# TRI-ML/packnet-sfm

Measured on AMD Instinct MI355X. Metric: images/sec PackNet01 self-sup train 192x640, higher is better.
Workload: dtype f32; 1 GPU; PackNet01(1A)+PoseNet self-supervised train step (fwd+photometric loss+bwd+allreduce+Adam), KITTI-shaped 192x640 triplets, batch 4/GPU (BASELINE.json configs[1]); global_batch=4, parallelism=dp1, wgrad_side_stream=True, pose_branch_stream=True, tuning=shipped database (346 decisions) + autotune for unlisted shapes, step_launch=eager, devices_visible=1

## Files before the change

include/pnsfm.h:

```cpp
#ifndef PNSFM_H
#define PNSFM_H

#include <stddef.h>
#include <stdint.h>

#ifdef __cplusplus
extern "C" {
#endif

int pnsfm_version(void);
const char* pnsfm_last_error(void);
const char* pnsfm_build_target(void);

size_t pnsfm_conv2d_packed_elems_fwd(int Cin, int Cout, int ks);
size_t pnsfm_conv2d_packed_elems_bwd(int Cin, int Cout, int ks);
int pnsfm_conv2d_pack_weights(const float* w, float* wp_fwd , float* wp_bwd ,
                              int Cin, int Cout, int ks, void* stream);
size_t pnsfm_conv2d_pack_item_bytes(void);
int pnsfm_conv2d_pack_item_fill(void* item_host, const float* w, float* wp_fwd, float* wp_bwd, int Cin, int Cout, int ks,
                                int first_block);
int pnsfm_conv2d_pack_table(const void* table_dev, int n_items, int total_blocks, void* stream);
int pnsfm_conv2d_forward(const float* x, const float* wp_fwd, const float* bias , float* y,
                         int B, int Cin, int Cout, int H, int W, int ks, void* stream);
int pnsfm_conv2d_backward_data(const float* dy, const float* wp_bwd, float* dx,
// ... 128 lines not shown
#define PNSFM_MAX_REGION_OPS 12
typedef struct {
  const float* src;
  float* dst;
  int n[4];
  long long src_stride[4];
  long long dst_stride[4];
  int op;
} pnsfm_region_op;
int pnsfm_region_ops(const void* ops_host, int n_ops, void* stream);

int pnsfm_upsample_nearest_forward(const float* x, float* y, int N, int h, int w, int s, void* stream);
int pnsfm_upsample_nearest_backward(const float* dy, float* dx, int N, int h, int w, int s, void* stream);

int pnsfm_loss_combine_forward(const float* const* photometric, int n, const float* const* smoothness, int ns, float weight,
                               float* out3, void* stream);
int pnsfm_loss_combine_backward(const float* g, int n, int ns, float weight, float* dout16, void* stream);

int pnsfm_pack_bias_eff_forward(const float* W2, const float* b2, const float* b3, float* Ssum, float* bias_eff, int C, int d,
                                int blk, void* stream);
int pnsfm_pack_bias_eff_backward(const float* g, const float* Ssum, const float* b3, const float* dWeff_full, float* db3, float* dW2,
                                 int C, int d, int D, int k, void* stream);

int pnsfm_adam_step(float* param, const float* grad, float* exp_avg, float* exp_avg_sq, size_t n,
                    float lr, float beta1, float beta2, float eps, float weight_decay, float grad_scale,
                    int step, void* stream);
int pnsfm_adam_flat_step(float* param, const float* grad, float* exp_avg, float* exp_avg_sq, size_t n, float* hp, void* stream);
int pnsfm_adam_flat_update(float* param, const float* grad, float* exp_avg, float* exp_avg_sq, size_t n, float* hp, int tick,
                           void* stream);
size_t pnsfm_adam_pack_item_bytes(void);
int pnsfm_adam_pack_item_fill(void* item_host, float* w, const float* g, float* m, float* v, const float* hp, float* wp_fwd,
                              float* wp_bwd, int Cin, int Cout, int ks, int first_block);
int pnsfm_adam_pack_table(const void* table_dev, int n_items, int total_blocks, void* stream);
size_t pnsfm_adam_seg_bytes(void);
int pnsfm_adam_seg_fill(void* seg_host, float* p, const float* g, float* m, float* v, const float* hp, size_t n, int first_block);
int pnsfm_adam_segments(const void* segs_dev, int nseg, int total_blocks, void* stream);

int pnsfm_stream_wait_stream(void* waiter, void* signaler);
int pnsfm_calib_mfma(float* sink, int blocks, int iters, void* stream);
int pnsfm_calib_copy(const float* src, float* dst, size_t n_floats, void* stream);
int pnsfm_prof_enable(int on);
int pnsfm_prof_reset(void);
int pnsfm_prof_collect(int kind, double* total_ms, double* total_flops, long long* launches);
int pnsfm_prof_dump(const char* path);

size_t pnsfm_sparse_compact_ws_ints(int ncell);
// ... 69 lines not shown
```

packnet-sfm_amd/csrc/api.hip:

```cpp
#include "pnsfm_common.h"
#include "../../include/pnsfm.h"

#include <cstdarg>
#include <cstdio>
#include <mutex>
#include <cstdlib>
#include <utility>
#include <vector>

namespace pnsfm {

static thread_local char g_err[512] = "";

void set_error(const char* fmt, ...) {
  va_list ap;
  va_start(ap, fmt);
  vsnprintf(g_err, sizeof(g_err), fmt, ap);
  va_end(ap);
}

int check_launch(const char* what) {
  int e = (int)hipGetLastError();
  if (e != 0) {
    set_error("%s: launch failed: %s", what, hipGetErrorString((hipError_t)e));
// ... 173 lines not shown
  if (hipGetDevice(&cur) != hipSuccess) { pnsfm::set_error("stream_wait_stream: hipGetDevice failed"); return -1; }
  const int dev = device_of(signaler, cur), dw = device_of(waiter, dev);
  if (dev < 0 || dev >= 64) { pnsfm::set_error("stream_wait_stream: bad device %d", dev); return -1; }
  if (dw != dev) { pnsfm::set_error("stream_wait_stream: the two streams live on different devices (%d, %d)", dw, dev); return -1; }
  struct DevGuard { int prev, now; DevGuard(int p, int n) : prev(p), now(n) { if (p != n) (void)hipSetDevice(n); } ~DevGuard() { if (prev != now) (void)hipSetDevice(prev); } } guard(cur, dev);
  hipEvent_t ev;
  {
    std::lock_guard<std::mutex> lk(mu);
    auto& r = ring[dev];
    if (r.size() < 256) {
      if (hipEventCreateWithFlags(&ev, hipEventDisableTiming) != hipSuccess) { pnsfm::set_error("stream_wait_stream: hipEventCreate failed"); return -1; }
      r.push_back(ev);
    } else {
      ev = r[next[dev]];
      next[dev] = (next[dev] + 1) % 256;
    }
  }
  if (hipEventRecord(ev, (hipStream_t)signaler) != hipSuccess) { pnsfm::set_error("stream_wait_stream: hipEventRecord failed"); return -1; }
  if (hipStreamWaitEvent((hipStream_t)waiter, ev, 0) != hipSuccess) { pnsfm::set_error("stream_wait_stream: hipStreamWaitEvent failed"); return -1; }
  return 0;
#endif
}

int pnsfm_prof_enable(int on) {
#ifndef PNSFM_EMU
  std::lock_guard<std::mutex> lk(pnsfm::g_prof_mu);
  pnsfm::g_prof_on = on != 0;
#else
  (void)on;
#endif
  return 0;
}

int pnsfm_prof_reset(void) {
#ifndef PNSFM_EMU
  std::lock_guard<std::mutex> lk(pnsfm::g_prof_mu);
  for (int k = 0; k < 2; ++k) {
    for (auto& r : pnsfm::g_recs[k]) {
      hipEventSynchronize(r.b);
      pnsfm::g_pool.push_back(r.a);
      pnsfm::g_pool.push_back(r.b);
    }
    pnsfm::g_recs[k].clear();
  }
#endif
  return 0;
// ... 43 lines not shown
```

packnet-sfm_amd/csrc/seq/pnsfm_seq.cpp:

```cpp
#include <torch/extension.h>

#include <cstdint>
#include <string>
#include <vector>

#include "../../../include/pnsfm.h"

namespace {

struct Abi {
  decltype(&pnsfm_last_error) last_error = nullptr;
  decltype(&pnsfm_conv2d_forward) conv2d_forward = nullptr;
  decltype(&pnsfm_conv2d_forward_cat) conv2d_forward_cat = nullptr;
  decltype(&pnsfm_conv2d_backward_data) conv2d_backward_data = nullptr;
  decltype(&pnsfm_conv2d_backward_data_add) conv2d_backward_data_add = nullptr;
  decltype(&pnsfm_conv2d_backward_weight) conv2d_backward_weight = nullptr;
  decltype(&pnsfm_conv2d_backward_weight_cat) conv2d_backward_weight_cat = nullptr;
  decltype(&pnsfm_groupnorm_act_forward) groupnorm_act_forward = nullptr;
  decltype(&pnsfm_groupnorm_act_backward) groupnorm_act_backward = nullptr;
  decltype(&pnsfm_stream_wait_stream) stream_wait_stream = nullptr;
  decltype(&pnsfm_region_ops) region_ops = nullptr;
  bool require_cuda = true;
  bool bound = false;
} g;

template <class F>
void take(F& slot, const py::dict& d, const char* name) {
  if (!d.contains(name)) throw std::runtime_error(std::string("pnsfm_seq.bind: missing symbol ") + name);
  slot = reinterpret_cast<F>(static_cast<uintptr_t>(d[name].cast<uint64_t>()));
}

void bind(const py::dict& addrs, bool require_cuda) {
  take(g.last_error, addrs, "pnsfm_last_error");
  take(g.conv2d_forward, addrs, "pnsfm_conv2d_forward");
  take(g.conv2d_forward_cat, addrs, "pnsfm_conv2d_forward_cat");
  take(g.conv2d_backward_data, addrs, "pnsfm_conv2d_backward_data");
  take(g.conv2d_backward_data_add, addrs, "pnsfm_conv2d_backward_data_add");
  take(g.conv2d_backward_weight, addrs, "pnsfm_conv2d_backward_weight");
  take(g.conv2d_backward_weight_cat, addrs, "pnsfm_conv2d_backward_weight_cat");
  take(g.groupnorm_act_forward, addrs, "pnsfm_groupnorm_act_forward");
  take(g.groupnorm_act_backward, addrs, "pnsfm_groupnorm_act_backward");
  take(g.stream_wait_stream, addrs, "pnsfm_stream_wait_stream");
  take(g.region_ops, addrs, "pnsfm_region_ops");
  g.require_cuda = require_cuda;
  g.bound = true;
}

void rc_check(int rc, const char* what) {
  if (rc != 0) throw std::runtime_error(std::string(what) + " failed (rc=" + std::to_string(rc) + "): " + (g.last_error ? g.last_error() : "?"));
}

void chk(const at::Tensor& t, const char* what, const at::Tensor* ref = nullptr) {
  if (g.require_cuda && !t.is_cuda())
    throw std::runtime_error(std::string("packnet_sfm HIP op got a ") + t.device().str() + " tensor (" + what +
                             "): the HIP kernels run on MI355X only, there is no CPU fallback");
  if (t.scalar_type() != at::kFloat) throw std::runtime_error(std::string("packnet_sfm HIP op needs float32 tensors (") + what + ")");
  if (!t.is_contiguous()) throw std::runtime_error(std::string("packnet_sfm HIP op needs contiguous tensors (") + what + ")");
  if (ref && t.device() != ref->device()) throw std::runtime_error("packnet_sfm HIP op got tensors on different devices");
}
const float* cptr(const at::Tensor& t) { return t.data_ptr<float>(); }
const float* cptr(const c10::optional<at::Tensor>& t) { return (t.has_value() && t->defined()) ? t->data_ptr<float>() : nullptr; }
float* mptr(at::Tensor& t) { return t.data_ptr<float>(); }
void* sp(uint64_t s) { return reinterpret_cast<void*>(static_cast<uintptr_t>(s)); }

void launch_conv_fwd(const std::vector<at::Tensor>& xs, const at::Tensor& wp, const c10::optional<at::Tensor>& bias, at::Tensor& y,
                     int Cout, int ks, uint64_t stream) {
// ... 203 lines not shown
      const auto& src = std::get<2>(it);
      const bool has_src = src.has_value() && src->defined();
      if (dst.scalar_type() != at::kFloat || (has_src && src->scalar_type() != at::kFloat)) throw std::runtime_error("region_ops needs float32 tensors");
      if (g.require_cuda && !dst.is_cuda())
        throw std::runtime_error("packnet_sfm HIP op got a " + dst.device().str() + " tensor: the HIP kernels run on MI355X only, there is no CPU fallback");
      if (dst.dim() > 4 || (has_src && src->sizes() != dst.sizes()) || dst.device() != ref.device())
        throw std::runtime_error("region_ops: windows must be <= 4-D, of equal shape, on one device");
      const int pad = 4 - (int)dst.dim();
      arr[k].dst = dst.data_ptr<float>();
      arr[k].src = has_src ? src->data_ptr<float>() : nullptr;
      arr[k].op = (int)std::get<0>(it);
      for (int d = 0; d < 4; ++d) {
        const int64_t nd = d < pad ? 1 : dst.size(d - pad);
        if (nd == 0) throw std::runtime_error("region_ops: empty window");
        arr[k].n[d] = (int)nd;
        arr[k].dst_stride[d] = d < pad ? 0 : dst.stride(d - pad);
        arr[k].src_stride[d] = (!has_src || d < pad) ? 0 : src->stride(d - pad);
      }
    }
    rc_check(g.region_ops(arr, (int)n, sp(stream)), "region_ops");
  }
}

}

PYBIND11_MODULE(TORCH_EXTENSION_NAME, m) {
  m.doc() = "packnet_sfm block sequencer: bodies of the hot autograd nodes as single calls over the C ABI of libpnsfm_hip.so";
  m.def("bind", &bind, py::arg("addresses"), py::arg("require_cuda"));
  m.def("conv_gn_act_forward", &conv_gn_act_forward);
  m.def("conv_gn_act_backward", &conv_gn_act_backward);
  m.def("conv2d_forward", &conv2d_forward);
  m.def("conv2d_backward", &conv2d_backward);
  m.def("gn_act_forward", &gn_act_forward);
  m.def("gn_act_backward", &gn_act_backward);
  m.def("region_ops", &region_ops);
}
```

packnet-sfm_amd/packnet_sfm/hip/_lib.py:

```python
import ctypes
import os

import torch

_HERE = os.path.dirname(os.path.abspath(__file__))
_CSRC = os.path.abspath(os.path.join(_HERE, "..", "..", "csrc"))
LIB_PATH = os.path.join(_CSRC, "libpnsfm_hip.so")

_p = ctypes.c_void_p
_i = ctypes.c_int
_f = ctypes.c_float
_sz = ctypes.c_size_t
_ll = ctypes.c_longlong
_d = ctypes.c_double

SIGNATURES = {
    "pnsfm_version": (_i, []),
    "pnsfm_last_error": (ctypes.c_char_p, []),
    "pnsfm_build_target": (ctypes.c_char_p, []),
    "pnsfm_conv2d_packed_elems_fwd": (_sz, [_i, _i, _i]),
    "pnsfm_conv2d_packed_elems_bwd": (_sz, [_i, _i, _i]),
    "pnsfm_conv2d_pack_weights": (_i, [_p, _p, _p, _i, _i, _i, _p]),
    "pnsfm_conv2d_pack_item_bytes": (_sz, []),
    "pnsfm_conv2d_pack_item_fill": (_i, [_p, _p, _p, _p, _i, _i, _i, _i]),
# ... 15 lines not shown
    "pnsfm_groupnorm_act_backward": (_i, [_p, _p, _p, _p, _p, _p, _p, _p, _p, _p, _p, _i, _i, _i, _i, _i, _p]),
    "pnsfm_set_gn_fused": (_i, [_i]),
    "pnsfm_space_to_depth": (_i, [_p, _p, _i, _i, _i, _i, _sz, _p]),
    "pnsfm_depth_to_space": (_i, [_p, _p, _i, _i, _i, _i, _p]),
    "pnsfm_conv3d_forward": (_i, [_p, _p, _p, _p, _i, _i, _i, _i, _i, _p]),
    "pnsfm_conv3d_backward_data": (_i, [_p, _p, _p, _i, _i, _i, _i, _i, _p]),
    "pnsfm_conv3d_backward_weight": (_i, [_p, _p, _p, _p, _p, _i, _i, _i, _i, _i, _p]),
    "pnsfm_set_pack3d_fold": (_i, [_i]),
    "pnsfm_conv3d_d2s_folded": (_i, [_p, _p, _i, _i]),
    "pnsfm_conv3d_forward_d2s": (_i, [_p, _p, _p, _p, _p, _i, _i, _i, _i, _i, _p]),
    "pnsfm_conv3d_rows_folded": (_i, [_p, _p, _i]),
    "pnsfm_conv3d_forward_rows": (_i, [_p, _p, _p, _p, _i, _i, _i, _i, _i, _i, _p]),
    "pnsfm_conv3d_backward_data_rows": (_i, [_p, _p, _p, _i, _i, _i, _i, _i, _i, _p]),
    "pnsfm_conv3d_backward_weight_rows": (_i, [_p, _p, _p, _p, _i, _i, _i, _i, _i, _i, _p]),
    "pnsfm_invdepth_act_forward": (_i, [_p, _p, _sz, _f, _p]),
    "pnsfm_invdepth_act_backward": (_i, [_p, _p, _p, _sz, _f, _p]),
    "pnsfm_pose_vec2mat_forward": (_i, [_p, _p, _i, _p]),
    "pnsfm_upsample_nearest_forward": (_i, [_p, _p, _i, _i, _i, _i, _p]),
    "pnsfm_upsample_nearest_backward": (_i, [_p, _p, _i, _i, _i, _i, _p]),
    "pnsfm_loss_combine_forward": (_i, [_p, _i, _p, _i, _f, _p, _p]),
    "pnsfm_loss_combine_backward": (_i, [_p, _i, _i, _f, _p, _p]),
    "pnsfm_pack_bias_eff_forward": (_i, [_p, _p, _p, _p, _p, _i, _i, _i, _p]),
    "pnsfm_pack_bias_eff_backward": (_i, [_p, _p, _p, _p, _p, _p, _i, _i, _i, _i, _p]),
    "pnsfm_pose_vec2mat_backward": (_i, [_p, _p, _p, _i, _p]),
    "pnsfm_supervised_loss_forward": (_i, [_p, _p, _p, _p, _sz, _i, _i, _p]),
    "pnsfm_supervised_loss_backward": (_i, [_p, _p, _p, _p, _p, _sz, _i, _i, _p]),
    "pnsfm_invdepth_conv_forward": (_i, [_p, _p, _p, _p, _i, _i, _i, _i, _f, _p]),
    "pnsfm_invdepth_conv_backward": (_i, [_p, _p, _p, _p, _p, _p, _i, _i, _i, _i, _p]),
    "pnsfm_view_synthesis_forward": (_i, [_p, _p, _p, _p, _p, _p, _i, _i, _i, _i, _i, _p]),
    "pnsfm_view_synthesis_backward": (_i, [_p, _p, _p, _p, _p, _p, _p, _p, _i, _i, _i, _i, _i, _p]),
    "pnsfm_photometric_forward": (_i, [_p, _p, _p, _p, _p, _p, _i, _i, _i, _i, _f, _f, _f, _i, _i, _f, _p]),
    "pnsfm_photometric_backward": (_i, [_p, _p, _p, _p, _f, _p, _i, _i, _i, _i, _f, _f, _f, _i, _i, _i, _p]),
    "pnsfm_smoothness_norm_forward": (_i, [_p, _p, _p, _p, _i, _i, _i, _p]),
    "pnsfm_smoothness_norm_backward": (_i, [_p, _p, _p, _p, _p, _i, _i, _i, _p]),
    "pnsfm_region_ops": (_i, [_p, _i, _p]),
    "pnsfm_conv2d_packed_elems_h16": (_sz, [_i, _i, _i]),
    "pnsfm_set_h16_max_split": (_i, [_i]),
    "pnsfm_conv2d_pack_weights_h16": (_i, [_p, _i, _p, _i, _i, _i, _p]),
    "pnsfm_conv2d_forward_h16": (_i, [_p, _i, _p, _i, _p, _i, _p, _p, _p, _i, _i, _i, _i, _i, _p]),
    "pnsfm_groupnorm_act_forward_h16": (_i, [_p, _p, _p, _p, _p, _p, _p, _i, _i, _i, _i, _f, _i, _p]),
    "pnsfm_conv3d_forward_h16": (_i, [_p, _p, _p, _p, _i, _i, _i, _i, _i, _p]),
    "pnsfm_space_to_depth_h16": (_i, [_p, _p, _i, _i, _i, _i, _p]),
    "pnsfm_depth_to_space_h16": (_i, [_p, _p, _i, _i, _i, _i, _p]),
    "pnsfm_upsample_nearest_forward_h16": (_i, [_p, _p, _i, _i, _i, _i, _p]),
    "pnsfm_invdepth_conv_forward_h16": (_i, [_p, _p, _p, _p, _i, _i, _i, _i, _f, _p]),
    "pnsfm_region_ops_h16": (_i, [_p, _i, _p]),
# ... 104 lines not shown
```

packnet-sfm_amd/packnet_sfm/hip/_seq.py:

```python
import ctypes
import importlib.util
import os

from . import _lib

_HERE = os.path.dirname(os.path.abspath(__file__))
SEQ_PATH = os.path.join(_HERE, "_pnsfm_seq.so")
_SYMBOLS = ("pnsfm_last_error", "pnsfm_conv2d_forward", "pnsfm_conv2d_forward_cat", "pnsfm_conv2d_backward_data",
            "pnsfm_conv2d_backward_data_add", "pnsfm_conv2d_backward_weight", "pnsfm_conv2d_backward_weight_cat",
            "pnsfm_groupnorm_act_forward", "pnsfm_groupnorm_act_backward", "pnsfm_stream_wait_stream", "pnsfm_region_ops")
_ON = os.environ.get("PNSFM_SEQ", "1") != "0"
_MOD = None
_BOUND = None


def set_enabled(on):
    global _ON
    _ON = bool(on)


def enabled():
    return _ON


def _load():
    global _MOD
    if _MOD is None:
        if not os.path.exists(SEQ_PATH):
            raise ImportError("%s not found -- build it with `python __graft_entry__.py` (packnet-sfm_amd/csrc/build.py: build_seq); "
                              "PNSFM_SEQ=0 runs the pure-Python bodies instead" % SEQ_PATH)
        spec = importlib.util.spec_from_file_location("_pnsfm_seq", SEQ_PATH)
        mod = importlib.util.module_from_spec(spec)
        spec.loader.exec_module(mod)
# ... 16 lines not shown
```

packnet-sfm_amd/packnet_sfm/hip/functional.py:

```python
import contextlib
import os
import weakref

import torch
from torch.autograd import Function
from torch.autograd.function import once_differentiable

from . import ops
from . import _seq
from ._lib import HipError as _HipError

_WEIGHT_EPOCH = [0]


def bump_weight_epoch():
    _WEIGHT_EPOCH[0] += 1


def get_conv_math():
    from . import _lib
    return 'bx3' if _lib.get().pnsfm_get_conv_math() else 'f32'


def set_conv_math(mode):
# ... 862 lines not shown
        return Weff

    @staticmethod
    @once_differentiable
    def backward(ctx, g):
        W2pad, w3 = ctx.saved_tensors
        g = g.contiguous()
        _WgradStream.side_ok(*ctx.params)
        dW2 = dW3 = None
        if ctx.needs_input_grad[0]:
            dW2 = ops.conv3d_forward(g, w3, torch.zeros(w3.shape[0], device=g.device, dtype=g.dtype))[:, :, 1:-1, 1:-1].contiguous()
        if ctx.needs_input_grad[1]:
            dW3, _ = ops.conv3d_backward_weight(g, W2pad)
        return dW2, dW3, None


def compose_pack_weight(W2, W3):
    return ComposePackWeightFn.apply(W2, W3, torch.is_grad_enabled())


class ComposePackParamsFn(Function):

    @staticmethod
    def forward(ctx, W2, b2, W3, b3, recording=True):
        W2d, w3, b3d = W2.detach().contiguous(), W3.detach().contiguous(), b3.detach().contiguous()
        W2pad = torch.nn.functional.pad(W2d, (1, 1, 1, 1))
        Weff = ops.conv3d_backward_data(W2pad, w3)
        bias_eff, Ssum = ops.pack_bias_eff_forward(W2d, None if b2 is None else b2.detach().contiguous(), b3d)
        ctx.save_for_backward(W2pad, w3, b3d, Ssum)
        ctx.params = (W2, W3)
        ctx.k = W2.shape[-1]
        _WgradStream.note_use(recording, W2, W3)
        return Weff, bias_eff

    @staticmethod
    @once_differentiable
    def backward(ctx, gW, gb):
        W2pad, w3, b3, Ssum = ctx.saved_tensors
        _WgradStream.side_ok(*ctx.params)
        need_W2, need_b2, need_W3, need_b3 = ctx.needs_input_grad[:4]
        C = W2pad.shape[0]
        if gW is None:
            gW = W2pad.new_zeros((C, W2pad.shape[1] // w3.shape[0], ctx.k + 2, ctx.k + 2))
        if gb is None:
            gb = W2pad.new_zeros((C,))
        gW, gb = gW.contiguous(), gb.contiguous()
        dW2 = dW3 = db3 = None
        if need_W2 or need_b3:
            full = ops.conv3d_forward(gW, w3, None) if need_W2 else W2pad
            db3, dW2 = ops.pack_bias_eff_backward(gb, Ssum, b3, full, ctx.k, want_db3=need_b3, want_dW2=need_W2)
        if need_W3:
            dW3, _ = ops.conv3d_backward_weight(gW, W2pad)
        return dW2, (gb if need_b2 else None), dW3, db3, None


def compose_pack_params(W2, b2, W3, b3):
    return ComposePackParamsFn.apply(W2, b2, W3, b3, torch.is_grad_enabled())


def _R(op, dst, src=None):
    return (op, dst, src)


def _border_split_fwd(P, S, lr_t, run):
    B, C, h, w = P.shape
    tb = P.new_empty((2 * B, C, S, w))
    lr = P.new_empty((2 * B, C, S, h)) if lr_t else P.new_empty((2 * B, C, h, S))
    lrv = lr.transpose(2, 3) if lr_t else lr
    run([_R(ops.REGION_COPY, tb[:B], P[:, :, :S]), _R(ops.REGION_COPY, tb[B:], P[:, :, h - S:]),
         _R(ops.REGION_COPY, lrv[:B], P[:, :, :, :S]), _R(ops.REGION_COPY, lrv[B:], P[:, :, :, w - S:])])
    return tb, lr


def _strip_select_fwd(z, B, r, dim, run):
    n2 = 2 * r
    if dim == 2:
        out = z.new_empty((z.shape[0], z.shape[1], n2, z.shape[3]))
        run([_R(ops.REGION_COPY, out[:B], z[:B, :, :n2]), _R(ops.REGION_COPY, out[B:], z[B:, :, 1:])])
    else:
        out = z.new_empty((z.shape[0], z.shape[1], z.shape[2], n2))
# ... 792 lines not shown
```

packnet-sfm_amd/packnet_sfm/hip/ops.py:

```python
import ctypes
import threading

import torch

from . import _lib


try:
    _raw_stream = torch._C._cuda_getCurrentRawStream
except AttributeError:
    _raw_stream = None


_TLS = threading.local()


class stream_override:

    def __init__(self, raw, device_index=None):
        self.ov = (raw, device_index)

    def __enter__(self):
        self.prev = getattr(_TLS, 'ov', None)
        _TLS.ov = self.ov
# ... 1223 lines not shown
        chunk = items[i0:i0 + MAX_REGION_OPS]
        arr = (_RegionOp * len(chunk))()
        for k, (op, dst, src) in enumerate(chunk):
            if dst.dtype != torch.float32 or (src is not None and src.dtype != torch.float32):
                raise RuntimeError("region_ops needs float32 tensors")
            if _lib.REQUIRE_CUDA and not dst.is_cuda:
                raise RuntimeError("packnet_sfm HIP op got a %s tensor: the HIP kernels run on MI355X only, there is no CPU fallback" % dst.device)
            if dst.dim() > 4 or (src is not None and tuple(src.shape) != tuple(dst.shape)) or dst.device != ref.device:
                raise RuntimeError("region_ops: windows must be <= 4-D, of equal shape, on one device")
            pad = 4 - dst.dim()
            shape = (1,) * pad + tuple(dst.shape)
            if 0 in shape:
                raise RuntimeError("region_ops: empty window")
            arr[k].dst = dst.data_ptr()
            arr[k].src = src.data_ptr() if src is not None else None
            arr[k].op = int(op)
            for d in range(4):
                arr[k].n[d] = shape[d]
                arr[k].dst_stride[d] = 0 if d < pad else dst.stride(d - pad)
                arr[k].src_stride[d] = 0 if (src is None or d < pad) else src.stride(d - pad)
        _lib.check(_lib.get().pnsfm_region_ops(ctypes.byref(arr), len(chunk), _stream(ref)), "region_ops")



def _h16(*tensors):
    for t in tensors:
        if t is not None and t.dtype != torch.float16:
            raise RuntimeError("packnet_sfm fp16 HIP op needs float16 tensors, got %s" % t.dtype)


def conv2d_pack_h16(w, out=None):
    _chk(w, out)
    if w.dtype not in (torch.float16, torch.float32):
        raise RuntimeError("conv2d_pack_h16: weight must be float16 or float32, got %s" % w.dtype)
    Cout, Cin, ks, _ = w.shape
    n = int(_lib.get().pnsfm_conv2d_packed_elems_h16(Cin, Cout, ks))
    if out is None or out.numel() != n or out.device != w.device:
        out = torch.empty(n, dtype=torch.float16, device=w.device)
    _h16(out)
    _lib.check(_lib.get().pnsfm_conv2d_pack_weights_h16(_ptr(w), 1 if w.dtype == torch.float32 else 0, _ptr(out), Cin, Cout, ks,
                                                         _stream(w)), "conv2d_pack_weights_h16")
    return out


def conv2d_forward_h16(xs, wp, bias, Cout, ks):
    xs = tuple(xs)
# ... 138 lines not shown
```

packnet-sfm_amd/packnet_sfm/networks/depth/PackNet01.py:

```python
import torch
import torch.nn as nn

from packnet_sfm.hip import functional as HF
from packnet_sfm.networks.layers.packnet.layers01 import Conv2D, InvDepth, PackLayerConv3d, ResidualBlock, UnpackLayerConv3d


class PackNet01(nn.Module):

    STEM_WIDTH = 64
    WIDTHS = (64, 64, 128, 256, 512)
    NUM_3D_FEAT = 8

    def __init__(self, dropout=None, version=None, **kwargs):
        super().__init__()
        if version is None or version[1:] not in ('A', 'B'):
            raise ValueError('Unknown PackNet version {}'.format(version))
        self.version = version[1:]
        concat = self.version == 'A'
        ni, no = self.STEM_WIDTH, 1
        n = list(self.WIDTHS)
        d3 = self.NUM_3D_FEAT
        blocks = [2, 2, 3, 3]
        pack_k = [5, 3, 3, 3, 3]
        if concat:
            dec_out = list(n)
            dec_in = [n[0] + ni + no, n[1] + n[0] + no, n[2] + n[1] + no, n[3] + n[2], n[4] + n[3]]
        else:
# ... 9 lines not shown
        unpack_in = [n[1], n[2], n[3], n[4], n[4]]
        for i in (4, 3, 2, 1, 0):
            setattr(self, 'unpack%d' % (i + 1), UnpackLayerConv3d(unpack_in[i], dec_out[i], 3, d=d3))
        for i in (4, 3, 2, 1, 0):
            setattr(self, 'iconv%d' % (i + 1), Conv2D(dec_in[i], n[i], 3, 1))
        for i in (3, 2, 1, 0):
            setattr(self, 'disp%d_layer' % (i + 1), InvDepth(n[i], out_channels=no))
        self.init_weights()

    def init_weights(self):
        for m in self.modules():
            if isinstance(m, (nn.Conv2d, nn.Conv3d)):
                nn.init.xavier_uniform_(m.weight)
                if m.bias is not None:
                    m.bias.data.zero_()

    def _merge(self, up, skip, disp=None):
        parts = (up, skip) if self.version == 'A' else (up + skip,)
        if disp is not None:
            parts = parts + (HF.upsample_nearest(disp, scale_factor=2),)
        return parts if len(parts) > 1 else parts[0]

    def forward(self, rgb):
        x = self.pre_calc(rgb)
        c1, x_s = self.conv1.forward_tap(x)
        x1p = self.pack1(c1)
        c2, x1p_s = self.conv2.forward_tap(x1p)
        x2p = self.pack2(c2)
        c3, x2p_s = self.conv3.forward_tap(x2p)
        x3p = self.pack3(c3)
        c4, x3p_s = self.conv4.forward_tap(x3p)
        x4p = self.pack4(c4)
        c5, x4p_s = self.conv5.forward_tap(x4p)
        x5p = self.pack5(c5)

        iconv5 = self.iconv5(self._merge(self.unpack5(x5p), x4p_s))
        iconv4 = self.iconv4(self._merge(self.unpack4(iconv5), x3p_s))
        up3, iconv4_t = self.unpack3.forward_tap(iconv4)
        disp4 = self.disp4_layer(iconv4_t)
        iconv3 = self.iconv3(self._merge(up3, x2p_s, disp4))
        up2, iconv3_t = self.unpack2.forward_tap(iconv3)
        disp3 = self.disp3_layer(iconv3_t)
        iconv2 = self.iconv2(self._merge(up2, x1p_s, disp3))
        up1, iconv2_t = self.unpack1.forward_tap(iconv2)
        disp2 = self.disp2_layer(iconv2_t)
        iconv1 = self.iconv1(self._merge(up1, x_s, disp2))
# ... 10 lines not shown
```

packnet-sfm_amd/packnet_sfm/networks/depth/PackNetSAN01.py:

```python
import torch
import torch.nn as nn

from packnet_sfm.hip import functional as HF
from packnet_sfm.networks.layers.minkowski_encoder import MinkowskiEncoder
from packnet_sfm.networks.layers.packnet.layers01 import Conv2D, InvDepth, PackLayerConv3d, ResidualBlock, UnpackLayerConv3d


class Encoder(nn.Module):
    def __init__(self, version, in_channels, ni, n1, n2, n3, n4, n5, pack_kernel, num_blocks, num_3d_feat, dropout):
        super().__init__()
        self.version = version
        n = [n1, n2, n3, n4, n5]
        self.pre_calc = Conv2D(in_channels, ni, 5, 1)
        for i in range(5):
            setattr(self, 'pack%d' % (i + 1), PackLayerConv3d(n[i], pack_kernel[i], d=num_3d_feat))
        self.conv1 = Conv2D(ni, n1, 7, 1)
        for i in range(4):
            setattr(self, 'conv%d' % (i + 2), ResidualBlock(n[i], n[i + 1], num_blocks[i], 1, dropout=dropout))

    def forward(self, rgb):
        x = self.pre_calc(rgb)
        x1p = self.pack1(self.conv1(x))
        x2p = self.pack2(self.conv2(x1p))
        x3p = self.pack3(self.conv3(x2p))
        x4p = self.pack4(self.conv4(x3p))
        x5p = self.pack5(self.conv5(x4p))
        return x5p, [x, x1p, x2p, x3p, x4p]


class Decoder(nn.Module):
    def __init__(self, version, out_channels, ni, n1, n2, n3, n4, n5, unpack_kernel, iconv_kernel, num_3d_feat):
        super().__init__()
        self.version = version
        n = [n1, n2, n3, n4, n5]
        nin = [n1 + ni + out_channels, n2 + n1 + out_channels, n3 + n2 + out_channels, n4 + n3, n5 + n4]
        unpack_in = [n2, n3, n4, n5, n5]
        for j, i in enumerate((4, 3, 2, 1, 0)):
            setattr(self, 'unpack%d' % (i + 1), UnpackLayerConv3d(unpack_in[i], n[i], unpack_kernel[j], d=num_3d_feat))
        for j, i in enumerate((4, 3, 2, 1, 0)):
            setattr(self, 'iconv%d' % (i + 1), Conv2D(nin[i], n[i], iconv_kernel[j], 1))
        self.unpack_disps = nn.PixelShuffle(2)
        self.unpack_disp4 = nn.Upsample(scale_factor=2, mode='nearest')
        self.unpack_disp3 = nn.Upsample(scale_factor=2, mode='nearest')
# ... 73 lines not shown
```

packnet-sfm_amd/packnet_sfm/networks/layers/packnet/layers01.py:

```python
import torch
import torch.nn as nn
import torch.nn.functional as F

from packnet_sfm.hip import functional as HF
from packnet_sfm.hip import ops as _ops


class _HipConv2d(nn.Conv2d):

    def __init__(self, in_channels, out_channels, kernel_size, stride=1):
        if stride != 1:
            raise NotImplementedError('the gfx950 conv kernel implements stride 1 only (all PackNet01 convs)')
        super().__init__(in_channels, out_channels, kernel_size=kernel_size, stride=stride)
        self._packed = HF.PackedConvWeight()

    def forward(self, x):
        if isinstance(x, (tuple, list)):
            return HF.conv2d_cat(tuple(x), self.weight, self.bias, self._packed)
        return HF.conv2d(x, self.weight, self.bias, self._packed)

    def forward_tap(self, x):
        return HF.conv2d_tap(x, self.weight, self.bias, self._packed)


# ... 103 lines not shown
        if r != 2:
            raise NotImplementedError('r=2 only')
        self.conv = Conv2D(in_channels, out_channels * (r ** 2), kernel_size, 1)

    def forward(self, x):
        return HF.depth_to_space(self.conv(x))


class PackLayerConv3d(nn.Module):

    collapse = 'auto'
    lr_transposed = True
    strip_frame_rows = True

    def __init__(self, in_channels, kernel_size, r=2, d=8):
        super().__init__()
        if r != 2 or d not in (4, 8):
            raise NotImplementedError('the gfx950 packing kernels implement r=2 and d in {4, 8} (PackNet01 / PackNetSlim01)')
        self.d = d
        self.conv = Conv2D(in_channels * (r ** 2) * d, in_channels, kernel_size, 1)
        self.conv3d = nn.Conv3d(1, d, kernel_size=(3, 3, 3), stride=(1, 1, 1), padding=(1, 1, 1))
        self._eff_packed = HF.PackedConvWeight(volatile=True)
        self._lr_packed = HF.PackedConvWeight()

    def _use_collapsed(self, h, w):
        k = self.conv.kernel_size
        r = k // 2
        if h < 2 * r + 1 or w < 2 * r + 1 or self.collapse is False:
            return False
        if self.collapse is True:
            return True
        orig = float(self.d) * k * k * h * w
        strips = float(self.d) * k * k * (2 * (2 * r) * w + 2 * h * (2 * r))
        return (k + 2) ** 2 * h * w + strips <= 0.7 * orig

    def _conv_reference_form(self, P):
        feats = HF.conv3d_1to8(P, self.conv3d.weight, self.conv3d.bias)
        return self.conv.conv_base(feats)

    def _conv_collapsed_h16(self, P):
        base = self.conv.conv_base
        W2, b2, W3, b3 = base.weight, base.bias, self.conv3d.weight, self.conv3d.bias
        HF._h16_params(W2, b2, W3, b3)
        return HF._h16_run(lambda P, *params: self._collapsed_h16_body(P), P, W2, b2, W3, b3)

    def _collapsed_h16_body(self, P):
        base = self.conv.conv_base
        W2, b2, W3, b3 = base.weight, base.bias, self.conv3d.weight, self.conv3d.bias
        key = tuple(None if t is None else HF.PackedConvWeight.key_of(t) for t in (W2, b2, W3, b3))
        with torch.no_grad():
            if self._eff_packed.key_h16 != key:
                W_eff, bias_eff = HF.compose_pack_params(W2.float(), None if b2 is None else b2.float(), W3.float(), b3.float())
                self._eff_packed.get_h16(W_eff, bias_eff, key=key, hold=(W2, b2, W3, b3))
            k = self.conv.kernel_size
            r, S = k // 2, 2 * (k // 2) + 1
            B = P.shape[0]
            lr_t = bool(self.lr_transposed)
            P_main, tb, lr = HF.pack_border_split(P, S, lr_t)
            y = HF.conv2d_h16_composed(P_main, None, None, self._eff_packed, key)
            o_tb = base(HF.strip_select(HF.conv3d_1to8(tb, W3, b3), B, r, 2))
            if lr_t:
                z = HF.conv3d_1to8(lr, W3.transpose(3, 4), b3)
                o_lr = HF.conv2d(HF.strip_select(z, B, r, 2), W2.transpose(2, 3), b2, self._lr_packed)
            else:
                o_lr = base(HF.strip_select(HF.conv3d_1to8(lr, W3, b3), B, r, 3))
            return HF.pack_border_paste(y, o_tb, o_lr, r, lr_t)

    def _conv_collapsed(self, P):
        if P.dtype == torch.float16:
            return self._conv_collapsed_h16(P)
        base = self.conv.conv_base
        W2, b2, W3, b3 = base.weight, base.bias, self.conv3d.weight, self.conv3d.bias
        k = self.conv.kernel_size
        r, S = k // 2, 2 * (k // 2) + 1
        B, _, h, w = P.shape
        W_eff, bias_eff = HF.compose_pack_params(W2, b2, W3, b3)
        lr_t = bool(self.lr_transposed)
        rows = bool(self.strip_frame_rows)
        P_main, tb, lr = HF.pack_border_split(P, S, lr_t)
        y = HF.conv2d(P_main, W_eff, bias_eff, self._eff_packed)
        s_tb = HF.conv3d_1to8_rows(tb, W3, b3, B, r)
        o_tb = HF.conv2d_rows(s_tb, W2, b2, base._packed, r) if rows else base(s_tb)
        if lr_t:
            z = HF.conv3d_1to8_rows(lr, W3.transpose(3, 4), b3, B, r)
            o_lr = (HF.conv2d_rows(z, W2.transpose(2, 3), b2, self._lr_packed, r) if rows else
                    HF.conv2d(z, W2.transpose(2, 3), b2, self._lr_packed))
        else:
            o_lr = base(HF.strip_select(HF.conv3d_1to8(lr, W3, b3), B, r, 3))
        return HF.pack_border_paste(y, o_tb, o_lr, r, lr_t, rows)

    def forward(self, x):
        P = HF.space_to_depth(x)
        y = self._conv_collapsed(P) if self._use_collapsed(P.shape[2], P.shape[3]) else self._conv_reference_form(P)
        norm = self.conv.normalize
        return HF.groupnorm_act(y, norm.weight, norm.bias, 16, norm.eps, _ops.ACT_ELU)


class UnpackLayerConv3d(nn.Module):

    def __init__(self, in_channels, out_channels, kernel_size, r=2, d=8):
        super().__init__()
        if r != 2 or d not in (4, 8):
            raise NotImplementedError('the gfx950 unpacking kernels implement r=2 and d in {4, 8} (PackNet01 / PackNetSlim01)')
        self.conv = Conv2D(in_channels, out_channels * (r ** 2) // d, kernel_size, 1)
        self.conv3d = nn.Conv3d(1, d, kernel_size=(3, 3, 3), stride=(1, 1, 1), padding=(1, 1, 1))

    def forward(self, x):
        return HF.conv3d_1to8_d2s(self.conv(x), self.conv3d.weight, self.conv3d.bias)

    def forward_tap(self, x):
        y, x_tap = self.conv.forward_tap(x)
        return HF.conv3d_1to8_d2s(y, self.conv3d.weight, self.conv3d.bias), x_tap


from packnet_sfm._merge import reference_fallback as _reference_fallback
__getattr__ = _reference_fallback(__name__, __file__)
```

Baseline: 178.6 images/sec.

## Precompute collapsed pack-layer weights on side stream at forward start

Adds a fused host entry point that pads W2, composes the effective weight and bias, and packs the forward/backward conv weights for each PackLayerConv3d in one call. At the start of the network forward these are issued for all pack layers on the wgrad side stream, and each layer waits on an event only just before its main conv. This moves per-layer weight composition and packing off the critical launch path so it overlaps with earlier layers. It adds persistent buffers and cross-stream dependencies, and relies on the layer's previous-call collapsed flag, so the first step takes the old path.

```diff
diff --git a/include/pnsfm.h b/include/pnsfm.h
--- a/include/pnsfm.h
+++ b/include/pnsfm.h
@@ -174,6 +174,24 @@
 int pnsfm_pack_bias_eff_backward(const float* g, const float* Ssum, const float* b3, const float* dWeff_full, float* db3, float* dW2,
                                  int C, int d, int D, int k, void* stream);
 
+typedef struct {
+  const float* W2;
+  const float* b2;
+  const float* W3;
+  const float* b3;
+  int C, D, d, k;
+  float* W2pad;
+  float* Weff;
+  float* bias_eff;
+  float* Ssum;
+  float* eff_fwd;
+  float* eff_bwd;
+  float* W2t;
+  float* lr_fwd;
+  float* lr_bwd;
+} pnsfm_pack_prepare_desc;
+int pnsfm_pack_prepare(const pnsfm_pack_prepare_desc* desc, void* stream, void* event );
+
 int pnsfm_adam_step(float* param, const float* grad, float* exp_avg, float* exp_avg_sq, size_t n,
                     float lr, float beta1, float beta2, float eps, float weight_decay, float grad_scale,
                     int step, void* stream);
diff --git a/packnet-sfm_amd/csrc/api.hip b/packnet-sfm_amd/csrc/api.hip
--- a/packnet-sfm_amd/csrc/api.hip
+++ b/packnet-sfm_amd/csrc/api.hip
@@ -219,6 +219,57 @@
 #endif
 }
 
+int pnsfm_pack_prepare(const pnsfm_pack_prepare_desc* p, void* stream, void* event) {
+  if (!p || !p->W2 || !p->W3 || !p->b3 || !p->W2pad || !p->Weff || !p->bias_eff || !p->Ssum || !p->eff_fwd || !p->eff_bwd) {
+    pnsfm::set_error("pack_prepare: null pointer");
+    return -1;
+  }
+  if (p->W2t && (!p->lr_fwd || !p->lr_bwd)) { pnsfm::set_error("pack_prepare: W2t without its packed buffers"); return -1; }
+  const int C = p->C, D = p->D, d = p->d, k = p->k, K2 = k + 2;
+  if (C < 1 || D < 1 || (d != 4 && d != 8) || (k != 1 && k != 3 && k != 5)) {
+    pnsfm::set_error("pack_prepare: unsupported shape (C=%d D=%d d=%d k=%d)", C, D, d, k);
+    return -1;
+  }
+  const long long DD = (long long)d * D;
+  pnsfm_region_op ops[2];
+  const int n_ops = p->W2t ? 2 : 1;
+  for (int i = 0; i < n_ops; ++i) {
+    ops[i].src = p->W2;
+    ops[i].op = 0;
+    ops[i].n[0] = C; ops[i].n[1] = (int)DD; ops[i].n[2] = k; ops[i].n[3] = k;
+    ops[i].src_stride[0] = DD * k * k; ops[i].src_stride[1] = k * k;
+  }
+  ops[0].dst = p->W2pad + K2 + 1;
+  ops[0].src_stride[2] = k; ops[0].src_stride[3] = 1;
+  ops[0].dst_stride[0] = DD * K2 * K2; ops[0].dst_stride[1] = K2 * K2; ops[0].dst_stride[2] = K2; ops[0].dst_stride[3] = 1;
+  if (p->W2t) {
+    ops[1].dst = p->W2t;
+    ops[1].src_stride[2] = 1; ops[1].src_stride[3] = k;
+    ops[1].dst_stride[0] = DD * k * k; ops[1].dst_stride[1] = k * k; ops[1].dst_stride[2] = k; ops[1].dst_stride[3] = 1;
+  }
+  int rc = pnsfm_region_ops(ops, n_ops, stream);
+  if (rc) return rc;
+  rc = pnsfm_conv3d_backward_data(p->W2pad, p->W3, p->Weff, C, D, K2, K2, d, stream);
+  if (rc) return rc;
+  rc = pnsfm_pack_bias_eff_forward(p->W2, p->b2, p->b3, p->Ssum, p->bias_eff, C, d, D * k * k, stream);
+  if (rc) return rc;
+  rc = pnsfm_conv2d_pack_weights(p->Weff, p->eff_fwd, p->eff_bwd, D, C, K2, stream);
+  if (rc) return rc;
+  if (p->W2t) {
+    rc = pnsfm_conv2d_pack_weights(p->W2t, p->lr_fwd, p->lr_bwd, (int)DD, C, k, stream);
+    if (rc) return rc;
+  }
+#ifndef PNSFM_EMU
+  if (event && hipEventRecord((hipEvent_t)event, (hipStream_t)stream) != hipSuccess) {
+    pnsfm::set_error("pack_prepare: hipEventRecord failed");
+    return -1;
+  }
+#else
+  (void)event;
+#endif
+  return 0;
+}
+
 int pnsfm_prof_enable(int on) {
 #ifndef PNSFM_EMU
   std::lock_guard<std::mutex> lk(pnsfm::g_prof_mu);
diff --git a/packnet-sfm_amd/csrc/seq/pnsfm_seq.cpp b/packnet-sfm_amd/csrc/seq/pnsfm_seq.cpp
--- a/packnet-sfm_amd/csrc/seq/pnsfm_seq.cpp
+++ b/packnet-sfm_amd/csrc/seq/pnsfm_seq.cpp
@@ -20,6 +20,7 @@
   decltype(&pnsfm_groupnorm_act_backward) groupnorm_act_backward = nullptr;
   decltype(&pnsfm_stream_wait_stream) stream_wait_stream = nullptr;
   decltype(&pnsfm_region_ops) region_ops = nullptr;
+  decltype(&pnsfm_pack_prepare) pack_prepare = nullptr;
   bool require_cuda = true;
   bool bound = false;
 } g;
@@ -42,6 +43,7 @@
   take(g.groupnorm_act_backward, addrs, "pnsfm_groupnorm_act_backward");
   take(g.stream_wait_stream, addrs, "pnsfm_stream_wait_stream");
   take(g.region_ops, addrs, "pnsfm_region_ops");
+  take(g.pack_prepare, addrs, "pnsfm_pack_prepare");
   g.require_cuda = require_cuda;
   g.bound = true;
 }
@@ -291,6 +293,38 @@
   }
 }
 
+void pack_prepare(const at::Tensor& W2, const c10::optional<at::Tensor>& b2, const at::Tensor& W3, const at::Tensor& b3, at::Tensor& W2pad,
+                  at::Tensor& Weff, at::Tensor& bias_eff, at::Tensor& Ssum, at::Tensor& eff_fwd, at::Tensor& eff_bwd,
+                  const c10::optional<at::Tensor>& W2t, const c10::optional<at::Tensor>& lr_fwd, const c10::optional<at::Tensor>& lr_bwd,
+                  const std::vector<int64_t>& packed_elems, uint64_t stream, uint64_t event) {
+  chk(W2, "W2"); chk(W3, "W3", &W2); chk(b3, "b3", &W2); chk(W2pad, "W2pad", &W2); chk(Weff, "Weff", &W2); chk(bias_eff, "bias_eff", &W2);
+  chk(Ssum, "Ssum", &W2); chk(eff_fwd, "eff_fwd", &W2); chk(eff_bwd, "eff_bwd", &W2);
+  const bool has_b2 = b2.has_value() && b2->defined(), lr = W2t.has_value() && W2t->defined();
+  if (has_b2) chk(*b2, "b2", &W2);
+  if (W2.dim() != 4 || W2.size(2) != W2.size(3)) throw std::runtime_error("pack_prepare: W2 must be [C, d*D, k, k]");
+  const int64_t C = W2.size(0), DD = W2.size(1), k = W2.size(2), d = b3.numel();
+  if (d < 1 || DD % d != 0 || W3.numel() != d * 27 || (has_b2 && b2->numel() != C)) throw std::runtime_error("pack_prepare: parameter shapes do not fit");
+  const int64_t D = DD / d, K2 = k + 2;
+  if (packed_elems.size() != 4) throw std::runtime_error("pack_prepare: four packed sizes expected");
+  if (W2pad.numel() != C * DD * K2 * K2 || Weff.numel() != C * D * K2 * K2 || bias_eff.numel() != C || Ssum.numel() != C * d ||
+      eff_fwd.numel() != packed_elems[0] || eff_bwd.numel() != packed_elems[1])
+    throw std::runtime_error("pack_prepare: a destination buffer has the wrong size");
+  pnsfm_pack_prepare_desc desc;
+  desc.W2 = cptr(W2); desc.b2 = has_b2 ? cptr(*b2) : nullptr; desc.W3 = cptr(W3); desc.b3 = cptr(b3);
+  desc.C = (int)C; desc.D = (int)D; desc.d = (int)d; desc.k = (int)k;
+  desc.W2pad = mptr(W2pad); desc.Weff = mptr(Weff); desc.bias_eff = mptr(bias_eff); desc.Ssum = mptr(Ssum);
+  desc.eff_fwd = mptr(eff_fwd); desc.eff_bwd = mptr(eff_bwd);
+  desc.W2t = nullptr; desc.lr_fwd = nullptr; desc.lr_bwd = nullptr;
+  if (lr) {
+    if (!lr_fwd.has_value() || !lr_fwd->defined() || !lr_bwd.has_value() || !lr_bwd->defined()) throw std::runtime_error("pack_prepare: W2t without its packed buffers");
+    chk(*W2t, "W2t", &W2); chk(*lr_fwd, "lr_fwd", &W2); chk(*lr_bwd, "lr_bwd", &W2);
+    if (W2t->numel() != W2.numel() || lr_fwd->numel() != packed_elems[2] || lr_bwd->numel() != packed_elems[3])
+      throw std::runtime_error("pack_prepare: a column-strip buffer has the wrong size");
+    desc.W2t = W2t->data_ptr<float>(); desc.lr_fwd = lr_fwd->data_ptr<float>(); desc.lr_bwd = lr_bwd->data_ptr<float>();
+  }
+  rc_check(g.pack_prepare(&desc, sp(stream), sp(event)), "pack_prepare");
+}
+
 }
 
 PYBIND11_MODULE(TORCH_EXTENSION_NAME, m) {
@@ -303,4 +337,5 @@
   m.def("gn_act_forward", &gn_act_forward);
   m.def("gn_act_backward", &gn_act_backward);
   m.def("region_ops", &region_ops);
-}
+  m.def("pack_prepare", &pack_prepare);
+}
diff --git a/packnet-sfm_amd/packnet_sfm/hip/_lib.py b/packnet-sfm_amd/packnet_sfm/hip/_lib.py
--- a/packnet-sfm_amd/packnet_sfm/hip/_lib.py
+++ b/packnet-sfm_amd/packnet_sfm/hip/_lib.py
@@ -61,6 +61,7 @@
     "pnsfm_loss_combine_backward": (_i, [_p, _i, _i, _f, _p, _p]),
     "pnsfm_pack_bias_eff_forward": (_i, [_p, _p, _p, _p, _p, _i, _i, _i, _p]),
     "pnsfm_pack_bias_eff_backward": (_i, [_p, _p, _p, _p, _p, _p, _i, _i, _i, _i, _p]),
+    "pnsfm_pack_prepare": (_i, [_p, _p, _p]),
     "pnsfm_pose_vec2mat_backward": (_i, [_p, _p, _p, _i, _p]),
     "pnsfm_supervised_loss_forward": (_i, [_p, _p, _p, _p, _sz, _i, _i, _p]),
     "pnsfm_supervised_loss_backward": (_i, [_p, _p, _p, _p, _p, _sz, _i, _i, _p]),
diff --git a/packnet-sfm_amd/packnet_sfm/hip/_seq.py b/packnet-sfm_amd/packnet_sfm/hip/_seq.py
--- a/packnet-sfm_amd/packnet_sfm/hip/_seq.py
+++ b/packnet-sfm_amd/packnet_sfm/hip/_seq.py
@@ -8,7 +8,7 @@
 SEQ_PATH = os.path.join(_HERE, "_pnsfm_seq.so")
 _SYMBOLS = ("pnsfm_last_error", "pnsfm_conv2d_forward", "pnsfm_conv2d_forward_cat", "pnsfm_conv2d_backward_data",
             "pnsfm_conv2d_backward_data_add", "pnsfm_conv2d_backward_weight", "pnsfm_conv2d_backward_weight_cat",
-            "pnsfm_groupnorm_act_forward", "pnsfm_groupnorm_act_backward", "pnsfm_stream_wait_stream", "pnsfm_region_ops")
+            "pnsfm_groupnorm_act_forward", "pnsfm_groupnorm_act_backward", "pnsfm_stream_wait_stream", "pnsfm_region_ops", "pnsfm_pack_prepare")
 _ON = os.environ.get("PNSFM_SEQ", "1") != "0"
 _MOD = None
 _BOUND = None
diff --git a/packnet-sfm_amd/packnet_sfm/hip/functional.py b/packnet-sfm_amd/packnet_sfm/hip/functional.py
--- a/packnet-sfm_amd/packnet_sfm/hip/functional.py
+++ b/packnet-sfm_amd/packnet_sfm/hip/functional.py
@@ -908,11 +908,14 @@
 class ComposePackParamsFn(Function):
 
     @staticmethod
-    def forward(ctx, W2, b2, W3, b3, recording=True):
+    def forward(ctx, W2, b2, W3, b3, recording=True, prep=None):
         W2d, w3, b3d = W2.detach().contiguous(), W3.detach().contiguous(), b3.detach().contiguous()
-        W2pad = torch.nn.functional.pad(W2d, (1, 1, 1, 1))
-        Weff = ops.conv3d_backward_data(W2pad, w3)
-        bias_eff, Ssum = ops.pack_bias_eff_forward(W2d, None if b2 is None else b2.detach().contiguous(), b3d)
+        if prep is not None:
+            W2pad, Weff, bias_eff, Ssum = (t.detach() for t in (prep.W2pad, prep.Weff, prep.bias_eff, prep.Ssum))
+        else:
+            W2pad = torch.nn.functional.pad(W2d, (1, 1, 1, 1))
+            Weff = ops.conv3d_backward_data(W2pad, w3)
+            bias_eff, Ssum = ops.pack_bias_eff_forward(W2d, None if b2 is None else b2.detach().contiguous(), b3d)
         ctx.save_for_backward(W2pad, w3, b3d, Ssum)
         ctx.params = (W2, W3)
         ctx.k = W2.shape[-1]
@@ -937,11 +940,109 @@
             db3, dW2 = ops.pack_bias_eff_backward(gb, Ssum, b3, full, ctx.k, want_db3=need_b3, want_dW2=need_W2)
         if need_W3:
             dW3, _ = ops.conv3d_backward_weight(gW, W2pad)
-        return dW2, (gb if need_b2 else None), dW3, db3, None
-
-
-def compose_pack_params(W2, b2, W3, b3):
-    return ComposePackParamsFn.apply(W2, b2, W3, b3, torch.is_grad_enabled())
+        return dW2, (gb if need_b2 else None), dW3, db3, None, None
+
+
+def compose_pack_params(W2, b2, W3, b3, prep=None):
+    return ComposePackParamsFn.apply(W2, b2, W3, b3, torch.is_grad_enabled(), prep)
+
+
+_PACK_PREPARE = os.environ.get('PNSFM_PACK_PREPARE', '1') != '0'
+
+
+def set_pack_prepare(on):
+    global _PACK_PREPARE
+    prev, _PACK_PREPARE = _PACK_PREPARE, bool(on)
+    return prev
+
+
+def pack_prepare_on():
+    return _PACK_PREPARE
+
+
+def prepare_stream(device):
+    return _WgradStream.get(device)
+
+
+class _PreparedPacked:
+
+    def __init__(self, wp_fwd, wp_bwd):
+        self.wp_fwd, self.wp_bwd = wp_fwd, wp_bwd
+
+    def get(self, weight, need_bwd):
+        return self.wp_fwd, (self.wp_bwd if need_bwd else None)
+
+
+class PackPrepared:
+
+    def __init__(self):
+        self.key = None
+        self.sig = None
+        self.event = None
+        self.lr = False
+
+    def _alloc(self, W2, d, lr):
+        C, DD, k, _ = W2.shape
+        sig = (tuple(W2.shape), d, W2.device, lr)
+        if self.sig == sig:
+            return
+        D = DD // d
+        new = lambda *shape: torch.empty(shape, dtype=torch.float32, device=W2.device)
+        self.sizes = ops.pack_prepare_sizes(C, D, d, k)
+        self.W2pad = torch.zeros((C, DD, k + 2, k + 2), dtype=torch.float32, device=W2.device)
+        self.Weff, self.bias_eff, self.Ssum = new(C, D, k + 2, k + 2), new(C), new(C, d)
+        self.eff = _PreparedPacked(new(self.sizes[0]), new(self.sizes[1]))
+        self.W2t = new(C, DD, k, k) if lr else None
+        self.lr_cache = _PreparedPacked(new(self.sizes[2]), new(self.sizes[3])) if lr else None
+        self.event = torch.cuda.Event() if W2.is_cuda else None
+        self._event_raw = 0
+        if W2.is_cuda:
+            for t in (self.W2pad, self.Weff, self.bias_eff, self.Ssum, self.eff.wp_fwd, self.eff.wp_bwd, self.W2t) + \
+                    (() if self.lr_cache is None else (self.lr_cache.wp_fwd, self.lr_cache.wp_bwd)):
+                if t is not None:
+                    t.record_stream(prepare_stream(W2.device))
+        self.sig, self.lr, self.key = sig, lr, None
+
+    def __reduce__(self):
+        return (PackPrepared, ())
+
+    @staticmethod
+    def key_for(W2, b2, W3, b3, lr):
+        return tuple(None if t is None else PackedConvWeight.key_of(t) for t in (W2, b2, W3, b3)) + (bool(lr),)
+
+    def issue(self, W2, b2, W3, b3, lr):
+        if W2.dtype != torch.float32 or not W2.is_contiguous() or not W3.is_contiguous():
+            return
+        key = self.key_for(W2, b2, W3, b3, lr)
+        if self.key == key:
+            return
+        self.key = None
+        dev = W2.device
+        with torch.cuda.device(dev) if dev.type == 'cuda' else contextlib.nullcontext():
+            self._alloc(W2, b3.numel(), bool(lr))
+            side_raw = 0
+            if dev.type == 'cuda':
+                side = prepare_stream(dev)
+                if not self._event_raw:
+                    self.event.record(side)
+                    self._event_raw = int(self.event.cuda_event)
+                side_raw = side.cuda_stream
+                ops.stream_wait_stream(side_raw, ops.launch_stream_raw(dev))
+            ops.pack_prepare(W2.detach(), None if b2 is None else b2.detach().contiguous(), W3.detach(), b3.detach().contiguous(),
+                             self.W2pad, self.Weff, self.bias_eff, self.Ssum, self.eff.wp_fwd, self.eff.wp_bwd, self.W2t,
+                             None if self.lr_cache is None else self.lr_cache.wp_fwd, None if self.lr_cache is None else self.lr_cache.wp_bwd,
+                             self.sizes, side_raw, self._event_raw)
+        self._src = tuple(None if t is None else t.detach() for t in (W2, b2, W3, b3))
+        self.key = key
+
+    def take(self, W2, b2, W3, b3, lr):
+        if self.key is None or self.key != self.key_for(W2, b2, W3, b3, lr):
+            return None
+        return self
+
+    def wait(self, device):
+        if self.event is not None:
+            torch.cuda.current_stream(device).wait_event(self.event)
 
 
 def _R(op, dst, src=None):
diff --git a/packnet-sfm_amd/packnet_sfm/hip/ops.py b/packnet-sfm_amd/packnet_sfm/hip/ops.py
--- a/packnet-sfm_amd/packnet_sfm/hip/ops.py
+++ b/packnet-sfm_amd/packnet_sfm/hip/ops.py
@@ -1269,6 +1269,42 @@
         _lib.check(_lib.get().pnsfm_region_ops(ctypes.byref(arr), len(chunk), _stream(ref)), "region_ops")
 
 
+class _PackPrepareDesc(ctypes.Structure):
+    _fields_ = [(n, ctypes.c_void_p) for n in ('W2', 'b2', 'W3', 'b3')] + [(n, ctypes.c_int) for n in ('C', 'D', 'd', 'k')] + \
+               [(n, ctypes.c_void_p) for n in ('W2pad', 'Weff', 'bias_eff', 'Ssum', 'eff_fwd', 'eff_bwd', 'W2t', 'lr_fwd', 'lr_bwd')]
+
+
+def pack_prepare_sizes(C, D, d, k):
+    return conv2d_packed_sizes(D, C, k + 2) + conv2d_packed_sizes(d * D, C, k)
+
+
+def pack_prepare(W2, b2, W3, b3, W2pad, Weff, bias_eff, Ssum, eff_fwd, eff_bwd, W2t, lr_fwd, lr_bwd, sizes, stream_raw, event_raw):
+    from . import _seq
+    sq = _seq.get()
+    if sq is not None:
+        sq.pack_prepare(W2, b2, W3, b3, W2pad, Weff, bias_eff, Ssum, eff_fwd, eff_bwd, W2t, lr_fwd, lr_bwd, list(sizes), stream_raw, event_raw)
+        return
+    ts = (W2, b2, W3, b3, W2pad, Weff, bias_eff, Ssum, eff_fwd, eff_bwd, W2t, lr_fwd, lr_bwd)
+    _chk(*ts); _f32(*ts)
+    C, DD, k, k2 = W2.shape
+    d = b3.numel()
+    if k != k2 or DD % d or W3.numel() != d * 27 or (b2 is not None and b2.numel() != C):
+        raise RuntimeError("pack_prepare: parameter shapes do not fit")
+    D, K2 = DD // d, k + 2
+    want = (C * DD * K2 * K2, C * D * K2 * K2, C, C * d, sizes[0], sizes[1])
+    if tuple(t.numel() for t in (W2pad, Weff, bias_eff, Ssum, eff_fwd, eff_bwd)) != want:
+        raise RuntimeError("pack_prepare: a destination buffer has the wrong size")
+    if W2t is not None and (lr_fwd is None or lr_bwd is None or (W2t.numel(), lr_fwd.numel(), lr_bwd.numel()) != (W2.numel(), sizes[2], sizes[3])):
+        raise RuntimeError("pack_prepare: a column-strip buffer has the wrong size")
+    desc = _PackPrepareDesc()
+    for n, t in zip(('W2', 'b2', 'W3', 'b3', 'W2pad', 'Weff', 'bias_eff', 'Ssum', 'eff_fwd', 'eff_bwd'), ts):
+        setattr(desc, n, None if t is None else t.data_ptr())
+    if W2t is not None:
+        desc.W2t, desc.lr_fwd, desc.lr_bwd = W2t.data_ptr(), lr_fwd.data_ptr(), lr_bwd.data_ptr()
+    desc.C, desc.D, desc.d, desc.k = C, D, d, k
+    _lib.check(_lib.get().pnsfm_pack_prepare(ctypes.byref(desc), ctypes.c_void_p(stream_raw), ctypes.c_void_p(event_raw)), "pack_prepare")
+
+
 
 def _h16(*tensors):
     for t in tensors:
diff --git a/packnet-sfm_amd/packnet_sfm/networks/depth/PackNet01.py b/packnet-sfm_amd/packnet_sfm/networks/depth/PackNet01.py
--- a/packnet-sfm_amd/packnet_sfm/networks/depth/PackNet01.py
+++ b/packnet-sfm_amd/packnet_sfm/networks/depth/PackNet01.py
@@ -2,7 +2,7 @@
 import torch.nn as nn
 
 from packnet_sfm.hip import functional as HF
-from packnet_sfm.networks.layers.packnet.layers01 import Conv2D, InvDepth, PackLayerConv3d, ResidualBlock, UnpackLayerConv3d
+from packnet_sfm.networks.layers.packnet.layers01 import Conv2D, InvDepth, PackLayerConv3d, ResidualBlock, UnpackLayerConv3d, prepare_packing
 
 
 class PackNet01(nn.Module):
@@ -58,6 +58,7 @@
         return parts if len(parts) > 1 else parts[0]
 
     def forward(self, rgb):
+        prepare_packing(self)
         x = self.pre_calc(rgb)
         c1, x_s = self.conv1.forward_tap(x)
         x1p = self.pack1(c1)
diff --git a/packnet-sfm_amd/packnet_sfm/networks/depth/PackNetSAN01.py b/packnet-sfm_amd/packnet_sfm/networks/depth/PackNetSAN01.py
--- a/packnet-sfm_amd/packnet_sfm/networks/depth/PackNetSAN01.py
+++ b/packnet-sfm_amd/packnet_sfm/networks/depth/PackNetSAN01.py
@@ -3,7 +3,7 @@
 
 from packnet_sfm.hip import functional as HF
 from packnet_sfm.networks.layers.minkowski_encoder import MinkowskiEncoder
-from packnet_sfm.networks.layers.packnet.layers01 import Conv2D, InvDepth, PackLayerConv3d, ResidualBlock, UnpackLayerConv3d
+from packnet_sfm.networks.layers.packnet.layers01 import Conv2D, InvDepth, PackLayerConv3d, ResidualBlock, UnpackLayerConv3d, prepare_packing
 
 
 class Encoder(nn.Module):
@@ -19,6 +19,7 @@
             setattr(self, 'conv%d' % (i + 2), ResidualBlock(n[i], n[i + 1], num_blocks[i], 1, dropout=dropout))
 
     def forward(self, rgb):
+        prepare_packing(self)
         x = self.pre_calc(rgb)
         x1p = self.pack1(self.conv1(x))
         x2p = self.pack2(self.conv2(x1p))
diff --git a/packnet-sfm_amd/packnet_sfm/networks/layers/packnet/layers01.py b/packnet-sfm_amd/packnet_sfm/networks/layers/packnet/layers01.py
--- a/packnet-sfm_amd/packnet_sfm/networks/layers/packnet/layers01.py
+++ b/packnet-sfm_amd/packnet_sfm/networks/layers/packnet/layers01.py
@@ -149,6 +149,8 @@
         self.conv3d = nn.Conv3d(1, d, kernel_size=(3, 3, 3), stride=(1, 1, 1), padding=(1, 1, 1))
         self._eff_packed = HF.PackedConvWeight(volatile=True)
         self._lr_packed = HF.PackedConvWeight()
+        self._prepared = HF.PackPrepared()
+        self._collapsed_last = False
 
     def _use_collapsed(self, h, w):
         k = self.conv.kernel_size
@@ -160,6 +162,14 @@
         orig = float(self.d) * k * k * h * w
         strips = float(self.d) * k * k * (2 * (2 * r) * w + 2 * h * (2 * r))
         return (k + 2) ** 2 * h * w + strips <= 0.7 * orig
+
+    def prepare(self, collapsed=None):
+        if collapsed is None:
+            collapsed = self._collapsed_last
+        if not (collapsed and HF.pack_prepare_on() and torch.is_grad_enabled()):
+            return
+        base = self.conv.conv_base
+        self._prepared.issue(base.weight, base.bias, self.conv3d.weight, self.conv3d.bias, bool(self.lr_transposed))
 
     def _conv_reference_form(self, P):
         feats = HF.conv3d_1to8(P, self.conv3d.weight, self.conv3d.bias)
@@ -201,26 +211,41 @@
         k = self.conv.kernel_size
         r, S = k // 2, 2 * (k // 2) + 1
         B, _, h, w = P.shape
-        W_eff, bias_eff = HF.compose_pack_params(W2, b2, W3, b3)
         lr_t = bool(self.lr_transposed)
+        prep = self._prepared.take(W2, b2, W3, b3, lr_t) if (HF.pack_prepare_on() and torch.is_grad_enabled()) else None
+        W_eff, bias_eff = HF.compose_pack_params(W2, b2, W3, b3, prep)
         rows = bool(self.strip_frame_rows)
         P_main, tb, lr = HF.pack_border_split(P, S, lr_t)
-        y = HF.conv2d(P_main, W_eff, bias_eff, self._eff_packed)
+        if prep is not None:
+            prep.wait(P.device)
+        y = HF.conv2d(P_main, W_eff, bias_eff, self._eff_packed if prep is None else prep.eff)
+        lr_packed = self._lr_packed if prep is None else prep.lr_cache
         s_tb = HF.conv3d_1to8_rows(tb, W3, b3, B, r)
         o_tb = HF.conv2d_rows(s_tb, W2, b2, base._packed, r) if rows else base(s_tb)
         if lr_t:
             z = HF.conv3d_1to8_rows(lr, W3.transpose(3, 4), b3, B, r)
-            o_lr = (HF.conv2d_rows(z, W2.transpose(2, 3), b2, self._lr_packed, r) if rows else
-                    HF.conv2d(z, W2.transpose(2, 3), b2, self._lr_packed))
+            o_lr = (HF.conv2d_rows(z, W2.transpose(2, 3), b2, lr_packed, r) if rows else
+                    HF.conv2d(z, W2.transpose(2, 3), b2, lr_packed))
         else:
             o_lr = base(HF.strip_select(HF.conv3d_1to8(lr, W3, b3), B, r, 3))
         return HF.pack_border_paste(y, o_tb, o_lr, r, lr_t, rows)
 
     def forward(self, x):
         P = HF.space_to_depth(x)
-        y = self._conv_collapsed(P) if self._use_collapsed(P.shape[2], P.shape[3]) else self._conv_reference_form(P)
+        collapsed = self._use_collapsed(P.shape[2], P.shape[3])
+        if P.dtype == torch.float32:
+            self._collapsed_last = collapsed
+        y = self._conv_collapsed(P) if collapsed else self._conv_reference_form(P)
         norm = self.conv.normalize
         return HF.groupnorm_act(y, norm.weight, norm.bias, 16, norm.eps, _ops.ACT_ELU)
+
+
+def prepare_packing(net):
+    if not (HF.pack_prepare_on() and torch.is_grad_enabled()):
+        return
+    for m in net.modules():
+        if isinstance(m, PackLayerConv3d):
+            m.prepare()
 
 
 class UnpackLayerConv3d(nn.Module):
```

After: 179.6 images/sec, median of 6. No clear change (+0.6%).
